# PRiME-project/PRiMEStereoMatch

Measured on AMD Instinct MI355X. Metric: cost-volume voxels/s (CVC+CVF+WTA), higher is better.
Workload: dtype f32; 1 GPU; synthetic 1920x1080 pair, D=256, float32 (BASELINE configs[3]); W=1920, H=1080, D=256, parallelism=1 GPU, kernel_variant=0, lr_check_on_gpu=False, batch=1, ranks=1, same_device=False, frames_in_flight=1

## Files before the change

### include/primesm_hip.h

```cpp
#ifndef PRIMESM_HIP_H
#define PRIMESM_HIP_H

#include <stddef.h>
#include <stdint.h>

#ifdef __cplusplus
extern "C" {
#endif

#define PSM_ABI_VERSION 1

typedef struct psm_ctx psm_ctx;

enum { PSM_F32 = 0, PSM_U8 = 1 };
enum { PSM_IMG_U8 = 0, PSM_IMG_F32 = 1 };
enum { PSM_LEFT = 0, PSM_RIGHT = 1 };
enum { PSM_STAGE_CVC = 0, PSM_STAGE_CVF = 1, PSM_STAGE_DISPSEL = 2, PSM_STAGE_PP = 3,
       PSM_STAGE_COUNT = 4 };
enum { PSM_K_PREP = 0, PSM_K_CVC = 1, PSM_K_GUIDE = 2, PSM_K_CVF_A = 3, PSM_K_CVF_B = 4,
       PSM_K_WTA = 5, PSM_K_MERGE = 6, PSM_K_BOX = 7, PSM_K_LRC = 8, PSM_K_CVF_F = 9, PSM_K_FGF = 10, PSM_K_WMF = 11,
       PSM_K_JWMF = 12, PSM_K_COUNT = 13 };
enum {
    PSM_OPT_ASYNC = 0,
    PSM_OPT_KERNEL_VARIANT = 1,
    PSM_OPT_PROFILE = 2,
    PSM_OPT_SEG_ROWS = 3,
    PSM_OPT_WAVES = 4,
    PSM_OPT_FLAGS = 5,
    PSM_OPT_GRAPH = 6,
    PSM_OPT_GATHER_STAGED = 7,
    PSM_OPT_FRAMES_IN_FLIGHT = 8
};

enum psm_flag {
    PSM_FLAG_MATERIALISE_COSTS = 128,
    PSM_FLAG_FGF_STORE = 4096,
    PSM_FLAG_STORE_FILTERED = 8192,
    PSM_FLAG_TWO_PHASE_ON = 1048576,
    PSM_FLAG_TWO_PHASE_OFF = 2097152,
    PSM_FLAG_WMF_DATAFLOW = 4194304,
    PSM_FLAG_WMF_TWO_SWEEPS = 8388608,
    PSM_FLAG_WMF_NO_CACHE = 16777216,
    PSM_FLAG_F32_TOL = 33554432,
    PSM_FLAG_FMA_SOLVE = 67108864,
    PSM_FLAGS_ALL = 128 | 4096 | 8192 | 1048576 | 2097152 | 4194304 | 8388608 | 16777216 | 33554432 | 67108864
};

int psm_device_count(void);

int psm_create(psm_ctx **out, int width, int height, int max_disp, int dtype, int device);

int psm_create_shard(psm_ctx **out, int width, int height, int max_disp, int d_begin, int d_end,
                     int dtype, int device);
int psm_create_shard_strided(psm_ctx **out, int width, int height, int max_disp, int d_first, int d_step,
// ... 189 lines not shown
```

### primestereomatch_amd/capi.py

```python
from __future__ import annotations

import ctypes as C
import os

_HERE = os.path.dirname(os.path.abspath(__file__))
LIB_PATH = os.path.join(_HERE, "lib", "libprimesm_hip.so")

PSM_F32, PSM_U8 = 0, 1
PSM_IMG_U8, PSM_IMG_F32 = 0, 1
PSM_LEFT, PSM_RIGHT = 0, 1
PSM_STAGE_CVC, PSM_STAGE_CVF, PSM_STAGE_DISPSEL, PSM_STAGE_PP = 0, 1, 2, 3
(PSM_K_PREP, PSM_K_CVC, PSM_K_GUIDE, PSM_K_CVF_A, PSM_K_CVF_B, PSM_K_WTA, PSM_K_MERGE, PSM_K_BOX,
 PSM_K_LRC, PSM_K_CVF_F, PSM_K_FGF, PSM_K_WMF, PSM_K_JWMF) = range(13)
(PSM_OPT_ASYNC, PSM_OPT_KERNEL_VARIANT, PSM_OPT_PROFILE, PSM_OPT_SEG_ROWS, PSM_OPT_WAVES, PSM_OPT_FLAGS, PSM_OPT_GRAPH,
 PSM_OPT_GATHER_STAGED, PSM_OPT_FRAMES_IN_FLIGHT) = range(9)
PSM_FLAG_MATERIALISE_COSTS, PSM_FLAG_FGF_STORE, PSM_FLAG_STORE_FILTERED = 128, 4096, 8192
PSM_FLAG_TWO_PHASE_ON, PSM_FLAG_TWO_PHASE_OFF = 1048576, 2097152
PSM_FLAG_WMF_DATAFLOW, PSM_FLAG_WMF_TWO_SWEEPS, PSM_FLAG_WMF_NO_CACHE = 4194304, 8388608, 16777216
PSM_FLAG_F32_TOL = 33554432
PSM_PP_LR_CHECK, PSM_PP_FILL, PSM_PP_WGT_MEDIAN = 1, 2, 4
PSM_FLAG_FMA_SOLVE = 67108864
PSM_SCORE_GIF, PSM_SCORE_SGM, PSM_SCORE_SGM_INT = 0, 1, 2
PSM_MASK_NONE, PSM_MASK_NONOCC, PSM_MASK_DISC = 0, 1, 2
PSM_SCORE_FLAT = 1
PSM_DEPTH_GIF, PSM_DEPTH_SGM = 0, 1
PSM_DEPTH_XYZ, PSM_DEPTH_Z, PSM_DEPTH_CLOUD = 1, 2, 4
PSM_DEPTH_USE_MASK = 1
PSM_DEPTH_VOID = 0x7FC00000
PSM_WLS_GIF, PSM_WLS_SGM = 0, 1
PSM_WLS_USE_MASK, PSM_WLS_CONFIDENCE = 1, 2
PSM_WLS_CONF_LR, PSM_WLS_CONF_VAR = 1, 2
PSM_WLS_VOID = 0x7FC00000


class Score(C.Structure):
    _fields_ = [("min_val", C.c_int32), ("max_val", C.c_int32), ("pixels", C.c_uint32), ("bad", C.c_uint32),
                ("err_sum", C.c_uint64), ("unit", C.c_int32), ("flags", C.c_uint32)]

# ... 179 lines not shown
```

### primestereomatch_amd/csrc/psm_api_core.cpp

```cpp
#include "psm_ctx.h"

#include <chrono>
#include <cstdarg>
#include <cstdio>
#include <cstring>

using namespace psm;

namespace {
std::string g_create_error;
}

namespace psm {

double now_us()
{
    using namespace std::chrono;
    return duration_cast<duration<double, std::micro>>(steady_clock::now().time_since_epoch()).count();
}

int fail(psm_ctx *c, const char *fmt, ...)
{
    char buf[512];
    va_list ap;
// ... 387 lines not shown
        if (value < 0) return fail(c, "psm_set_option: seg_rows %d < 0", value);
        c->march.seg_rows = value; return 0;
    case PSM_OPT_WAVES:
        if (value != 1 && value != 2 && value != 4 && value != 8) return fail(c, "psm_set_option: waves %d not in {1,2,4,8}", value);
        c->march.waves = value; return 0;
    case PSM_OPT_FLAGS:
        if (value & ~PSM_FLAGS_ALL) return fail(c, "psm_set_option: unknown flag bits 0x%x", value & ~PSM_FLAGS_ALL);
        if (c->dtype == PSM_U8) value &= ~(PSM_FLAG_FMA_SOLVE | PSM_FLAG_F32_TOL);
        if ((value & PSM_FLAG_F32_TOL) && (value & PSM_FLAG_FMA_SOLVE))
            return fail(c, "psm_set_option: PSM_FLAG_F32_TOL and PSM_FLAG_FMA_SOLVE exclude each other (one arithmetic variant at a time)");
        if ((value ^ c->march.flags) & PSM_FLAG_FMA_SOLVE) c->guid_rows = Rows{};
        c->march.flags = value; return 0;
    case PSM_OPT_GRAPH:
#ifdef PSM_EXPERIMENTS
        c->opt_graph = value != 0; return 0;
#else
        if (value != 0) return fail(c, "psm_set_option: PSM_OPT_GRAPH is not part of the product library (hipGraph replay of a batch measured slower than its plain launches)");
        return 0;
#endif
    case PSM_OPT_GATHER_STAGED: c->opt_gather_staged = value != 0; return 0;
    case PSM_OPT_FRAMES_IN_FLIGHT:
        if (value < 1 || value > 64) return fail(c, "psm_set_option: frames in flight %d not in [1, 64]", value);
        c->march.inflight = value; return 0;
    default: return fail(c, "psm_set_option: unknown option %d", option);
    }
}

int psm_set_stream(psm_ctx *c, void *hip_stream)
{
    if (!c) return 1;
    if (bind(c)) return 1;
    if (c->shared) return fail(c, "psm_set_stream: the context shares its streams with a batch (psm_share_streams)");
    PSM_HIP(c, hipStreamSynchronize(c->stream));
    c->stream = hip_stream ? (hipStream_t)hip_stream : c->own_stream;
    return 0;
}

int psm_synchronize(psm_ctx *c)
{
    if (!c) return 1;
    if (bind(c)) return 1;
    PSM_HIP(c, hipStreamSynchronize(c->stream));
    if (c->copy_stream) PSM_HIP(c, hipStreamSynchronize(c->copy_stream));
    if (c->down_stream && c->down_stream != c->copy_stream) PSM_HIP(c, hipStreamSynchronize(c->down_stream));
    return 0;
}
// ... 249 lines not shown
```

### primestereomatch_amd/csrc/psm_kernels.h

```cpp
#pragma once
#include <hip/hip_runtime.h>
#include <stdint.h>
#include "psm_live.h"
#include "psm_wm_sched.h"
#include "psm_wls_tab.h"

namespace psm {

struct Guidance {
    float4 *g1;
    float4 *g2;
    float4 *g3;
    float2 *g4;
};

struct March {
    int seg_rows;
    int waves;
    int flags;
    int dstep = 1;
    int inflight = 1;
    int ybeg = 0, yend = 0;
    int y0(int H) const { (void)H; return yend > ybeg ? ybeg : 0; }
    int y1(int H) const { return yend > ybeg ? yend : H; }
    int rows(int H) const { return y1(H) - y0(H); }
};

struct PcPair {
    const void *raw[2];
    Guidance g[2];
    uint8_t *p4[2];
    void *scratch;
    long long *keys;
    uint8_t *maps;
};
template <typename R> struct Recs { const R *host, *dev; int n; };
template <typename R, int N = 1> struct RecVal { R r[N]; };
template <typename R> using RecTab = const R *;
template <typename R> __device__ __forceinline__ const R &rec(const R *tab, unsigned i) { return tab[i]; }
template <typename R, int N> __device__ __forceinline__ const R &rec(const RecVal<R, N> &v, unsigned i) { return v.r[N == 1 ? 0 : i]; }
template <typename T>
__device__ __forceinline__ T *sgm_global(T *const &slot) { return (T *)*(__attribute__((address_space(1))) T *const *)(const void *)&slot; }
template <typename T> struct RecArg { using type = T; };
// ... 26 lines not shown
using PcTab = RecTab<PcPair>;
void launch_merge_batch(hipStream_t s, const Recs<PcPair> &q, int W, int H);

void launch_copy_bytes(hipStream_t s, void *dst, const void *src, size_t bytes);
void launch_range_f32(hipStream_t s, const float *p, size_t n, unsigned *out);
void launch_prep(hipStream_t s, const Recs<PcPair> &q, size_t pitch, int depth_f32, int W, int y0, int y1, bool u8_planes);
void launch_guidance(hipStream_t s, const Recs<PcPair> &q, int W, int H, int ybeg, int yend, bool fma, int src = 0, size_t pitch = 0);
void launch_cvc(hipStream_t s, const float4 *g1_base, const float4 *g1_other, float *vol, int W, int H,
                int d_begin, int Dloc, int right, int ybeg, int yend);
void launch_cvf_a(hipStream_t s, int variant, March m, const float *vol, float4 *ab, Guidance g, int W,
                  int H, int Dloc, int ybeg, int yend);
void launch_cvf_b_direct(hipStream_t s, const float4 *ab, float *vol, Guidance g, int W, int H, int Dloc);
void launch_cvf_fused(hipStream_t s, March m, const Recs<PcPair> &q, const float *vin, float *vout, int W, int H, int Dloc,
                      int ybeg, int yend, int d_begin, int cvc_mode, unsigned long long *ts = nullptr);
struct PcDev { int nxcd = 0, cus_per_xcd = 0; };
PcDev pc_dev();
enum { PC_STORE = 0, PC_PLANES = 1, PC_KEYS = 2, PC_BOTH = 4 };
struct PcPlan {
    int ngroups, nsegs, seg_rows, DC, nchunks, nbmax, nxcd;
    int cols;
    bool narrow;
    size_t rec_per_chunk;
    int rec_bytes;
    size_t scratch_bytes() const { return rec_per_chunk * (size_t)nchunks * rec_bytes; }
};
PcPlan pc_plan(int W, int rows, int Dloc, int seg_rows_opt, int form, int batch = 1, int inflight = 1);
PcPlan pc_plan_select(March m, int W, int H, int Dloc, int form, int npairs, bool batch);
int pc_seed_stride(int W, int rows, bool u8);
constexpr int PC_TS_SLOTS = 4096;
void launch_cvf_select(hipStream_t s, March m, const Recs<PcPair> &q, const float *vin, bool u8, int W, int H, int Dloc, int d_begin,
                       int cvc_mode, unsigned long long *ts = nullptr);
void launch_chunk_min(hipStream_t s, March m, const Recs<PcPair> &q, int W, int H, int Dloc);
void launch_cvf_select2(hipStream_t s, March m, const Recs<PcPair> &q, bool u8, int W, int H, int Dloc, int d_begin, unsigned long long *ts,
                        int sel, int step);
void launch_chunk_min2sides(hipStream_t s, March m, const Recs<PcPair> &q, int W, int H, int Dloc, bool to_maps, int d_begin, int sel, int step);
void launch_cvf_select_keys2(hipStream_t s, March m, const Recs<PcPair> &q, bool u8, int W, int H, int Dloc, int d_begin,
                             unsigned long long *ts, int sel, int step);
void launch_box8(hipStream_t s, int variant, March m, const float *vol, float *out, int W, int H, int Dloc);
void launch_wta(hipStream_t s, const float *vol, int W, int H, int d_begin, int Dloc, long long *keys,
                uint8_t *map);
void launch_merge(hipStream_t s, const long long *keys_all, size_t rank_stride, int nranks, int n,
                  uint8_t *map);

void launch_wgt_median(hipStream_t s, uint8_t *dis, const uint8_t *valid, const float4 *g1, int W, int H, int maxDis, int right,
                       int *nxt, int *prog, int *err);
struct WmSide {
// ... 261 lines not shown
```

### primestereomatch_amd/csrc/psm_pc.hip

```cpp
#include "psm_kernels.h"
#include "psm_cost.h"
#include "psm_dev.h"
#include "psm_live.h"
#include "../../include/primesm_hip.h"

#include <mutex>
#include <type_traits>

#include "psm_pc_debug.inc"

namespace psm {

typedef float f4v __attribute__((ext_vector_type(4)));

constexpr int PC_RING = 4;

template <int MODE, bool NARROW = false> struct PcLayout;
template <> struct PcLayout<0, false> { static constexpr int NA = 2, NB = 2, OUT_A = 52, OUT_B = 48, COLS = 96; };
template <> struct PcLayout<1, false> { static constexpr int NA = 2, NB = 2, OUT_A = 57, OUT_B = 54, COLS = 107; };
template <> struct PcLayout<2, false> : PcLayout<1, false> {};
template <> struct PcLayout<1, true> { static constexpr int NA = 1, NB = 1, OUT_A = 57, OUT_B = 50, COLS = 50; };
template <> struct PcLayout<2, true> : PcLayout<1, true> {};
constexpr int PC_K_LD_AUX = 0;
constexpr int PC_KEY_LD_AUX = 1;

typedef unsigned pc_u2 __attribute__((ext_vector_type(2)));
// ... 8 lines not shown
}
__device__ __forceinline__ float pc_load1_l2(__amdgpu_buffer_rsrc_t r, int voff, int soff)
{
    return __uint_as_float(__builtin_amdgcn_raw_buffer_load_b32(r, voff, soff, 16));
}
__device__ __forceinline__ float2 pc_load2(__amdgpu_buffer_rsrc_t r, int voff, int soff)
{
    const pc_u2 v = __builtin_amdgcn_raw_buffer_load_b64(r, voff, soff, 0);
    return make_float2(__uint_as_float(v.x), __uint_as_float(v.y));
}
__device__ __forceinline__ float4 pc_load4(__amdgpu_buffer_rsrc_t r, int voff, int soff)
{
    const pc_u4 v = __builtin_amdgcn_raw_buffer_load_b128(r, voff, soff, 0);
    return make_float4(__uint_as_float(v.x), __uint_as_float(v.y), __uint_as_float(v.z), __uint_as_float(v.w));
}

typedef unsigned pc_u3 __attribute__((ext_vector_type(3)));
__device__ __forceinline__ float3 pc_load3(__amdgpu_buffer_rsrc_t r, int voff, int soff)
{
    const pc_u3 v = __builtin_amdgcn_raw_buffer_load_b96(r, voff, soff, 0);
    return make_float3(__uint_as_float(v.x), __uint_as_float(v.y), __uint_as_float(v.z));
}

constexpr int PC_LIVE_MAX = 6;
struct PcLive {
    int on;
    int lo, full;
    int pre[2], nshort[2], tot[2];
    int cnt[2][PC_LIVE_MAX];
};
__host__ __device__ __forceinline__ int pc_live_count(const PcLive &lv, int side, int g)
{
    const int k = g - (side ? lv.pre[1] : lv.pre[0]), ns = side ? lv.nshort[1] : lv.nshort[0];
    int c = lv.full;
#pragma unroll
    for (int i = 0; i < PC_LIVE_MAX; ++i)
        if (i == k && i < ns) c = side ? lv.cnt[1][i] : lv.cnt[0][i];
    return c;
}
struct PcSel {
    int sel, step;
    int nxcd;
    int spread;
    unsigned long long rec_total;
    int dstep;
    PcLive live;
};
__device__ __forceinline__ int pc_spread(const PcSel &o, int n, int i)
{
    if (o.spread > 1) {
        int r = 0, base = 0;
        for (; r < o.spread; ++r) {
            const int cnt = (n - r + o.spread - 1) / o.spread;
            if (i < base + cnt) break;
            base += cnt;
        }
        i = (i - base) * o.spread + r;
    }
    return i;
}

template <bool VEC4, int CVC, int MODE, typename S, bool U8 = false, int VAR = 0, bool NARROW = false>
__global__ __launch_bounds__(64 * (PcLayout<MODE, NARROW>::NA + PcLayout<MODE, NARROW>::NB))
__attribute__((amdgpu_waves_per_eu(MODE == 2 ? 4 : 1, MODE == 2 ? 4 : 8)))
void k_cvf_pc(S src, const float *__restrict__ vin, float *__restrict__ vout, int W, int H, int Dloc, int ngroups, int nsegs, int seg_rows,
              int ybeg, int yend, int d_begin, int DC, int nbmax, PcSel dyn, unsigned long long *__restrict__ ts)
{
    constexpr bool TOL = VAR == 1, FMA = VAR == 2, TABLE = std::is_pointer<S>::value;
    static_assert(VAR >= 0 && VAR <= 2 && !(TOL && (U8 || MODE == 0)) && !(FMA && (U8 || TABLE)), "tolerance form: float select forms; FMA solve: float mode, single pair");
    static_assert(!TABLE || (CVC == 3 && MODE != 0), "batched launches: both volumes per launch, select forms");
    const bool right = CVC == 2 || (CVC == 3 && blockIdx.y == 1);
    const bool s1 = CVC == 3 && blockIdx.y == 1;
    const PcPair &pp = rec(src, blockIdx.z);
    const float4 *const G1 = s1 ? pp.g[1].g1 : pp.g[0].g1, *const G2 = s1 ? pp.g[1].g2 : pp.g[0].g2, *const G3 = s1 ? pp.g[1].g3 : pp.g[0].g3;
    const float2 *const G4 = s1 ? pp.g[1].g4 : pp.g[0].g4;
    const float4 *const Gother = s1 ? pp.g[0].g1 : pp.g[1].g1;
    if (U8) { vin = (const float *)pp.p4[0]; vout = (float *)pp.p4[1]; }
    float *const kcost = MODE == 1 ? (float *)((char *)pp.scratch + (s1 ? dyn.rec_total * 20 : 0))
                       : MODE == 2 ? (float *)(pp.keys + (s1 ? (size_t)W * H : 0)) : nullptr;
    unsigned *const kdisp = MODE == 1 ? (unsigned *)(kcost + 4 * dyn.rec_total) : nullptr;
    static_assert(!NARROW || (MODE != 0 && CVC == 3), "the narrow layout exists for the two-volume select forms");
    using L = PcLayout<MODE, NARROW>;
    constexpr int PC_NA = L::NA, PC_NB = L::NB, PC_OUT_A = L::OUT_A, PC_OUT_B = L::OUT_B, PC_COLS = L::COLS;
    constexpr int PC_MCOLS = PC_NA * PC_OUT_A;
    constexpr bool SCALED = MODE != 0;
    constexpr float QSCALE = SCALED ? 0x1p-12f : 1.0f;
#define PSM_BOX(N) (SCALED ? (float)(N) : box_out(N))
    static_assert(PC_MCOLS >= PC_COLS + 7 && PC_OUT_A <= 57 && PC_OUT_B <= 57 && (MODE != 0 || (PC_COLS % 4) == 0), "bad producer/consumer layout");
    __shared__ __attribute__((aligned(16))) float4 ring[PC_RING][4][PC_MCOLS];
    __shared__ __attribute__((aligned(16))) float qbuf[MODE == 0 ? 2 : 1][MODE == 0 ? 4 : 1][MODE == 0 ? PC_COLS : 4];
    int id = blockIdx.x;
    const int npairs = ngroups * nsegs;
    const PcLive &lv = dyn.live;
    const int ltot = s1 ? lv.tot[1] : lv.tot[0];
    const int nitems = nsegs * ltot;
    const int ipx = (nitems + dyn.nxcd - 1) / dyn.nxcd;
    const int xcd = id % dyn.nxcd, jj = id / dyn.nxcd;
    const int item = xcd * ipx + jj;
    if (jj >= ipx || item >= nitems) return;
    if (ts != nullptr && threadIdx.x == 0) {
        (void)__hip_atomic_fetch_min(ts, (unsigned long long)wall_clock64(), __ATOMIC_RELAXED, __HIP_MEMORY_SCOPE_AGENT);
        if (blockIdx.x == 0 && blockIdx.y == 0) ts[2 * PC_TS_SLOTS] = (unsigned long long)MODE;
    }
    const int seg = item / ltot;
    int g, gi = item - seg * ltot, gn = lv.full;
    {
        const int pre = s1 ? lv.pre[1] : lv.pre[0], ns = s1 ? lv.nshort[1] : lv.nshort[0];
        if (gi < pre * lv.full) { g = gi / lv.full; gi -= g * lv.full; }
        else {
            gi -= pre * lv.full;
            g = pre;
            bool found = false;
#pragma unroll
            for (int k = 0; k < PC_LIVE_MAX; ++k) {
                const int c = s1 ? lv.cnt[1][k] : lv.cnt[0][k];
                if (!found && k < ns) {
                    if (gi < c) { found = true; gn = c; }
                    else { gi -= c; ++g; }
                }
            }
            if (!found) { const int q = gi / lv.full; g += q; gi -= q * lv.full; }
        }
    }
    const int pair = seg * ngroups + g;
    const int ch = lv.lo + gi;
    const int sl0 = pc_sel_index(dyn.sel, dyn.step, MODE == 2 ? lv.lo + pc_spread(dyn, gn, gi) : ch);
    const int wave = __builtin_amdgcn_readfirstlane(threadIdx.x >> 6), lane = threadIdx.x & 63;
    const bool is_a = wave < PC_NA;
    const int xg = g * PC_COLS;
    const int xm0 = xg - 4;
    const int y0 = ybeg + seg * seg_rows, y1 = min(yend, y0 + seg_rows);
    const int mstart = max(0, y0 - 4);
    const int mend = min(H - 1, max(y1 + 2, 4 - y0));
    const int nbA = (mend - mstart + 1 + 3) >> 2;
    const int nf = (y1 - y0) + 7;
    const int nbB = (nf + 3) >> 2;
    const int iters = nbB + 3;
    const int i1 = ((lane + 1) & 63) << 2, i2 = ((lane + 2) & 63) << 2, i4 = ((lane + 4) & 63) << 2;
    (void)i1;
    const size_t HW = (size_t)H * W;

    PC_TRACE_BEGIN()
    int ds_lo = 0, ds_hi = MODE == 1 ? min(DC, Dloc - ch * DC) : 1;
    if (MODE == 1 && lv.on) {
        const PcOwn own = {1, d_begin, dyn.dstep, dyn.sel, dyn.step};
        while (ds_lo < ds_hi && pc_dead_at(own, right, xg, xg + PC_COLS - 1, W, ch * DC + ds_lo)) ++ds_lo;
        while (ds_hi > ds_lo && pc_dead_at(own, right, xg, xg + PC_COLS - 1, W, ch * DC + ds_hi - 1)) --ds_hi;
        if (ds_lo >= ds_hi) return;
    }
    bool first = true;
    int rb = 0;
    for (int ds = ds_lo; ds < ds_hi; ++ds) {
    const int sl = MODE == 1 ? pc_sel_index(dyn.sel, dyn.step, ch * DC + ds) : sl0;
    const bool last_slice = ds == ds_hi - 1;
// ... 376 lines not shown
        int gs = -1, ge = -1;
        for (int g = 0; g < ngroups; ++g) {
            const int xf = g * cols, xl = xf + cols - 1;
            const int L = pc_live_end(own, side, xf, xl, W, n);
            if ((L < n && !pc_dead_at(own, side, xf, xl, W, L)) || (L - 1 >= skip0 && pc_dead_at(own, side, xf, xl, W, L - 1))) return all;
            const int end = chunks ? (L + DC - 1) / DC : L, c = L > skip0 && end > lv.lo ? end - lv.lo : 0;
            lv.tot[side] += c;
            if (c == lv.full) continue;
            if (gs < 0) gs = g;
            ge = g;
        }
        if (gs < 0) continue;
        if (ge - gs + 1 > PC_LIVE_MAX) return all;
        lv.pre[side] = gs;
        lv.nshort[side] = ge - gs + 1;
        for (int g = gs; g <= ge; ++g) {
            const int L = pc_live_end(own, side, g * cols, g * cols + cols - 1, W, n), end = chunks ? (L + DC - 1) / DC : L;
            lv.cnt[side][g - gs] = L > skip0 && end > lv.lo ? end - lv.lo : 0;
        }
    }
    return lv;
}

PcPlan pc_plan(int W, int rows, int Dloc, int seg_rows_opt, int form, int batch, int inflight)
{
    const bool planes = (form & 3) == PC_PLANES, keys = (form & 3) == PC_KEYS;
    if (PSM_KNOB(planes ? "PSM_PC_SEGP" : "PSM_PC_SEGK", 0) > 0 && (planes || keys))
        seg_rows_opt = PSM_KNOB(planes ? "PSM_PC_SEGP" : "PSM_PC_SEGK", 0);
    const int sides = ((form & PC_BOTH) ? 2 : 1) * (batch > 1 ? batch : 1);
    const PcDev dev = pc_dev();
    PcPlan pl;
    pl.nxcd = dev.nxcd;
    constexpr int WIDE = PcLayout<1>::COLS, NARROW = PcLayout<1, true>::COLS;
    const bool select2 = (form & 3) != PC_STORE && (form & PC_BOTH);
    const int narrow_knob = PSM_KNOB("PSM_PC_NARROW", 0);
    pl.narrow = select2 && (narrow_knob ? narrow_knob == 1 : 2 * ((W + NARROW - 1) / NARROW) < 4 * ((W + WIDE - 1) / WIDE));
    const int cols = (form & 3) == PC_STORE ? PcLayout<0>::COLS : (pl.narrow ? NARROW : WIDE);
    pl.cols = cols;
    pl.ngroups = (W + cols - 1) / cols;
    const int kdiv = PSM_KNOB("PSM_PC_KDIV", rows < 128 ? 32 : 64);
    const int kmax = rows / kdiv > 1 ? rows / kdiv : 1;
    int dcs[5] = {1, 2, 4, 8, 16};
    int ndc = planes ? 5 : 1;
    if (planes && PSM_KNOB("PSM_PC_DC", 0) > 0) { dcs[0] = PSM_KNOB("PSM_PC_DC", 0); ndc = 1; }
    const long slots = PSM_KNOB("PSM_PC_SLOTS", (long)dev.cus_per_xcd * (keys ? 4 : 3) * (pl.narrow ? 2 : 1));
    const int conc = inflight > 1 ? inflight : 1;
    const int model_knob = PSM_KNOB("PSM_PC_MODEL", 0);
    const bool flow = model_knob ? model_knob == 1 : (sides * conc > 2 && (long)W * rows < 524288);
    auto cost_of = [&](int dc, int kk) -> long {
        const int nch = (Dloc + dc - 1) / dc;
        if (flow) {
            const double items = (double)sides * conc * pl.ngroups * kk * nch, len = dc * ((rows + kk - 1) / kk + 14) + 10.0;
            double c = items * len / ((double)slots * dev.nxcd) + 0.5 * len;
            if (planes && dc == 1) c *= 1.06;
            return (long)(c * 16.0);
        }
        const long per_xcd = ((long)sides * pl.ngroups * kk * nch + dev.nxcd - 1) / dev.nxcd;
        if (keys) {
            return (2 * ((per_xcd + slots - 1) / slots) + 3) * ((rows + kk - 1) / kk + 30) / 2;
        }
        const long rounds2 = 2 * ((per_xcd + slots - 1) / slots) + 1;
        long c = rounds2 * dc * ((rows + kk - 1) / kk + 14) / 2 + (planes ? 2L * sides * nch : 0);
        if (planes && dc == 1) c += (long)(0.06 * c * ((double)W * rows >= 2097152.0 ? 1.0 : (double)W * rows / 2097152.0));
        return c;
    };
    auto allowed = [&](int dc, int kk) { return (dc == dcs[0] || dc <= Dloc) && (seg_rows_opt <= 0 || kk == (rows + seg_rows_opt - 1) / seg_rows_opt); };
    long best = -1;
    for (int di = 0; di < ndc; ++di)
        for (int kk = 1; kk <= kmax && kk <= 32; ++kk)
            if (allowed(dcs[di], kk)) { const long c = cost_of(dcs[di], kk); if (best < 0 || c < best) best = c; }
    int bk = seg_rows_opt > 0 ? (rows + seg_rows_opt - 1) / seg_rows_opt : 1, bdc = dcs[0];
    for (int di = 0; di < ndc && best >= 0; ++di)
        for (int kk = 1; kk <= kmax && kk <= 32; ++kk)
            if (allowed(dcs[di], kk) && cost_of(dcs[di], kk) == best) { bk = kk; bdc = dcs[di]; di = ndc; break; }
    pl.seg_rows = seg_rows_opt > 0 ? seg_rows_opt : (rows + bk - 1) / bk;
    if (pl.seg_rows > rows) pl.seg_rows = rows;
    pl.nsegs = (rows + pl.seg_rows - 1) / pl.seg_rows;
    pl.DC = bdc;
    pl.nchunks = (Dloc + bdc - 1) / bdc;
    pl.nbmax = (pl.seg_rows + 7 + 3) / 4;
    pl.rec_per_chunk = (size_t)pl.ngroups * pl.nsegs * pl.nbmax * pl.cols;
    pl.rec_bytes = 20;
    return pl;
}

constexpr int PC_KEY_SPREAD = 4;

int pc_seed_stride(int W, int rows, bool u8)
{
    const int e = PSM_KNOB("PSM_PC_S", 0);
    if (e > 1) return e;
    if (rows < 200 || (u8 && (size_t)W * rows >= 1500000)) return 5;
    return 8;
}

static int pc_blocks(const PcPlan &pl, const PcLive &lv)
{
    const int items = pl.nsegs * (lv.tot[0] > lv.tot[1] ? lv.tot[0] : lv.tot[1]);
    return pl.nxcd * ((items + pl.nxcd - 1) / pl.nxcd);
}

struct PcArgs {
    Recs<PcPair> q;
    const float *vin;
    float *vout;
    int W, H, Dloc, ybeg, yend, d_begin;
    PcSel sel;
    unsigned long long *ts;
};

struct PcForm {
    int mode, cvc;
    bool u8;
    int var;
    bool narrow, vec4;
};

template <int V> using pc_int = std::integral_constant<int, V>;
template <int... Vs, class Fn> static void pc_pick(int v, Fn &&fn) { (void)((v == Vs && (fn(pc_int<Vs>{}), true)) || ...); }
template <class Fn> static void pc_pick_bool(bool b, Fn &&fn) { if (b) fn(std::true_type{}); else fn(std::false_type{}); }

static void pc_launch(hipStream_t s, const PcPlan &pl, dim3 grid, const PcArgs &a, const PcForm &f)
{
    using F = std::false_type;
    using T = std::true_type;
    const bool planes = f.mode == PC_PLANES;
    if (grid.x == 0) return;
    const PcVal val = {{a.q.host[0]}};
    const PcTab tab = a.q.dev;
    auto go = [&](auto V4, auto CV, auto MD, auto src, auto U, auto VR, auto NW) {
        using L = PcLayout<MD, NW>;
        hipLaunchKernelGGL(HIP_KERNEL_NAME(k_cvf_pc<V4, CV, MD, decltype(src), U, VR, NW>), grid, dim3(64 * (L::NA + L::NB)), 0, s, src, a.vin,
                           a.vout, a.W, a.H, a.Dloc, pl.ngroups, pl.nsegs, pl.seg_rows, a.ybeg, a.yend, a.d_begin, planes ? pl.DC : 1,
                           planes ? pl.nbmax : 0, a.sel, a.ts);
    };
    if (f.mode == PC_STORE)
        pc_pick_bool(f.vec4, [&](auto V4) { pc_pick<0, 1, 2>(f.cvc, [&](auto CV) {
            pc_pick<0, 2>(f.var, [&](auto VR) { go(V4, CV, pc_int<0>{}, val, F{}, VR, F{}); }); }); });
    else if (f.cvc != 3)
        pc_pick<0, 1, 2>(f.cvc, [&](auto CV) {
            if constexpr (CV != 0) if (f.u8) return go(F{}, CV, pc_int<1>{}, val, T{}, pc_int<0>{}, F{});
            pc_pick<0, 2>(f.var, [&](auto VR) { go(F{}, CV, pc_int<1>{}, val, F{}, VR, F{}); });
        });
    else
        pc_pick<1, 2>(f.mode, [&](auto MD) { pc_pick_bool(f.narrow, [&](auto NW) {
            if (tab) pc_pick_bool(f.u8, [&](auto U) { go(F{}, pc_int<3>{}, MD, tab, U, pc_int<0>{}, NW); });
            else if (f.u8) go(F{}, pc_int<3>{}, MD, val, T{}, pc_int<0>{}, NW);
            else pc_pick<0, 1, 2>(f.var, [&](auto VR) { go(F{}, pc_int<3>{}, MD, val, F{}, VR, NW); });
        }); });
}

static int pc_var(March m, bool u8)
{
    return u8 ? 0 : (m.flags & PSM_FLAG_FMA_SOLVE) ? 2 : (m.flags & PSM_FLAG_F32_TOL) ? 1 : 0;
}

static void pc_chunk_min(hipStream_t s, March m, const PcPlan &pl, int W, int H, int sides, const Recs<PcPair> &q, const PcLive &lv, bool to_maps)
{
    rec_launch(s, k_chunk_min<PcVal>, k_chunk_min<PcTab>, dim3((unsigned)((pl.rec_per_chunk + 255) / 256), sides, q.n),
               dim3(256), 0, q, pl.nchunks, pl.ngroups * pl.nsegs, pl.nbmax, pl.ngroups, pl.seg_rows, W, H, m.y0(H), m.y1(H), to_maps ? 1 : 0,
               pl.cols, lv);
}

void launch_cvf_fused(hipStream_t s, March m, const Recs<PcPair> &q, const float *vin, float *vout, int W, int H, int Dloc,
                      int ybeg, int yend, int d_begin, int cvc_mode, unsigned long long *ts)
{
    if (yend <= ybeg) return;
    const PcPlan pl = pc_plan(W, yend - ybeg, Dloc, m.seg_rows, PC_STORE);
    const PcLive lv = pc_live(W, pl.cols, pl.ngroups, Dloc, 1, false, PcOwn{});
    const PcArgs a = {q, vin, vout, W, H, Dloc, ybeg, yend, d_begin, PcSel{0, 1, pl.nxcd, 0, 0, 1, lv}, ts};
    const int cvc = cvc_mode == 1 || cvc_mode == 2 ? cvc_mode : 0;
    pc_launch(s, pl, dim3(pc_blocks(pl, lv)), a, {PC_STORE, cvc, false, (m.flags & PSM_FLAG_FMA_SOLVE) ? 2 : 0, false, (W & 3) == 0});
}

void launch_cvf_select(hipStream_t s, March m, const Recs<PcPair> &q, const float *vin, bool u8, int W, int H, int Dloc, int d_begin,
                       int cvc_mode, unsigned long long *ts)
{
    const PcPlan pl = pc_plan(W, m.rows(H), Dloc, m.seg_rows, PC_PLANES);
    const int cvc = cvc_mode == 1 || cvc_mode == 2 ? cvc_mode : 0;
    const PcLive lv = pc_live(W, pl.cols, pl.ngroups, Dloc, pl.DC, true, PcOwn{});
    const PcArgs a = {q, vin, nullptr, W, H, Dloc, m.y0(H), m.y1(H), d_begin, PcSel{0, 1, pl.nxcd, 0, pl.rec_per_chunk * pl.nchunks, 1, lv}, ts};
    pc_launch(s, pl, dim3(pc_blocks(pl, lv)), a, {PC_PLANES, cvc, u8 && cvc != 0, (m.flags & PSM_FLAG_FMA_SOLVE) ? 2 : 0, false, false});
}

void launch_chunk_min(hipStream_t s, March m, const Recs<PcPair> &q, int W, int H, int Dloc)
{
    const PcPlan pl = pc_plan(W, m.rows(H), Dloc, m.seg_rows, PC_PLANES);
    pc_chunk_min(s, m, pl, W, H, 1, q, pc_live(W, pl.cols, pl.ngroups, Dloc, pl.DC, true, PcOwn{}), false);
}

static PcOwn pc_own(March m, int d_begin, int sel, int step) { return PcOwn{1, d_begin, m.dstep, sel, step}; }
PcPlan pc_plan_select(March m, int W, int H, int Dloc, int form, int npairs, bool batch)
{
    return pc_plan(W, m.rows(H), Dloc, m.seg_rows, form | PC_BOTH, npairs, batch ? 1 : m.inflight);
}

void launch_cvf_select2(hipStream_t s, March m, const Recs<PcPair> &q, bool u8, int W, int H, int Dloc, int d_begin, unsigned long long *ts,
                        int sel, int step)
{
    const PcPlan pl = pc_plan_select(m, W, H, Dloc, PC_PLANES, q.n, q.dev != nullptr);
    const PcLive lv = pc_live(W, pl.cols, pl.ngroups, Dloc, pl.DC, true, pc_own(m, d_begin, sel, step));
    const PcArgs a = {q, nullptr, nullptr, W, H, Dloc, m.y0(H), m.y1(H), d_begin,
                      PcSel{sel, step, pl.nxcd, 0, pl.rec_per_chunk * pl.nchunks, m.dstep, lv}, ts};
    pc_launch(s, pl, dim3(pc_blocks(pl, lv), 2, q.n), a, {PC_PLANES, 3, u8, pc_var(m, u8), pl.narrow, false});
}

void launch_chunk_min2sides(hipStream_t s, March m, const Recs<PcPair> &q, int W, int H, int Dloc, bool to_maps, int d_begin, int sel, int step)
{
    const PcPlan pl = pc_plan_select(m, W, H, Dloc, PC_PLANES, q.n, q.dev != nullptr);
    const PcLive lv = pc_live(W, pl.cols, pl.ngroups, Dloc, pl.DC, true, pc_own(m, d_begin, sel, step));
    pc_chunk_min(s, m, pl, W, H, 2, q, lv, to_maps);
}

void launch_cvf_select_keys2(hipStream_t s, March m, const Recs<PcPair> &q, bool u8, int W, int H, int Dloc, int d_begin,
                             unsigned long long *ts, int sel, int step)
{
    const PcPlan pl = pc_plan_select(m, W, H, Dloc, PC_KEYS, q.n, q.dev != nullptr);
    const PcLive lv = pc_live(W, pl.cols, pl.ngroups, Dloc, 1, false, pc_own(m, d_begin, sel, step));
    const PcArgs a = {q, nullptr, nullptr, W, H, Dloc, m.y0(H), m.y1(H), d_begin,
                      PcSel{sel, step, pl.nxcd, PSM_KNOB("PSM_PC_SPREAD", PC_KEY_SPREAD), 0, m.dstep, lv}, ts};
    pc_launch(s, pl, dim3(pc_blocks(pl, lv), 2, q.n), a, {PC_KEYS, 3, u8, pc_var(m, u8), pl.narrow, false});
}

}

extern "C" int psm_debug_pc_dead(int right, int xfirst, int xlast, int W, int dg, int dprev)
{
    return psm::pc_dead(right, xfirst, xlast, W, dg, dprev) ? 1 : 0;
}

extern "C" int psm_debug_pc_items(int W, int rows, int nsl, int form, int d_begin, int dstep, int sel, int step, int *out)
{
    using namespace psm;
    if (!out || W < 1 || rows < 1 || nsl < 1 || dstep < 1 || form < PC_STORE || form > PC_KEYS) return 1;
    March m = {};
    m.dstep = dstep;
    m.yend = rows;
    PcOwn own = pc_own(m, d_begin, sel, step);
    if (form == PC_STORE) own.on = 0;
    const PcPlan pl = form == PC_STORE ? pc_plan(W, rows, nsl, 0, PC_STORE) : pc_plan_select(m, W, rows, nsl, form, 1, false);
    const bool chunks = form == PC_PLANES;
    const PcLive lv = pc_live(W, pl.cols, pl.ngroups, nsl, chunks ? pl.DC : 1, chunks, own);
    int slices[2] = {0, 0};
    for (int side = 0; side < 2; ++side)
        for (int g = 0; g < pl.ngroups; ++g)
            for (int j = 0; j < nsl; ++j)
                slices[side] += pc_dead_at(own, side, g * pl.cols, g * pl.cols + pl.cols - 1, W, j) ? 0 : 1;
    const int v[12] = {pl.ngroups, pl.nsegs, pl.DC, pl.cols, lv.tot[0], lv.tot[1], pl.ngroups * (chunks ? pl.nchunks : nsl),
                       slices[0], slices[1], pc_blocks(pl, lv), lv.lo, 0};
    for (int i = 0; i < 12; ++i) out[i] = v[i];
    return 0;
}

extern "C" int psm_debug_pc_group_items(int W, int rows, int nsl, int form, int d_begin, int dstep, int sel, int step, int side, int g,
                                        int *out)
{
    using namespace psm;
    if (!out || W < 1 || rows < 1 || nsl < 1 || dstep < 1 || form < PC_PLANES || form > PC_KEYS || side < 0 || side > 1 || g < 0) return 1;
    March m = {};
    m.dstep = dstep;
    m.yend = rows;
    const PcPlan pl = pc_plan_select(m, W, rows, nsl, form, 1, false);
    if (g >= pl.ngroups) return 1;
    const bool chunks = form == PC_PLANES;
    const PcLive lv = pc_live(W, pl.cols, pl.ngroups, nsl, chunks ? pl.DC : 1, chunks, pc_own(m, d_begin, sel, step));
    out[0] = lv.lo;
    out[1] = pc_live_count(lv, side, g);
    return 0;
}
```

Measured before the change: 167.9 billion voxels/s.

## Schedule key-select blocks with a two-tier segment split to balance the tail round

Adds a host-computed schedule for the single-pair key-select CVF launch. Both sides are merged into one flattened item list, spread across XCDs, and a tail set of items is split into finer row segments so the last wave of blocks fills the slots. A cost model picks between the plain split and the two-tier split, and a new option or env knob can force a cut. The kernel decodes its item from the schedule, which adds per-block index math and shorter segments with extra halo rows in the tail.

```diff
diff --git a/include/primesm_hip.h b/include/primesm_hip.h
--- a/include/primesm_hip.h
+++ b/include/primesm_hip.h
@@ -29,7 +29,8 @@
     PSM_OPT_FLAGS = 5,
     PSM_OPT_GRAPH = 6,
     PSM_OPT_GATHER_STAGED = 7,
-    PSM_OPT_FRAMES_IN_FLIGHT = 8
+    PSM_OPT_FRAMES_IN_FLIGHT = 8,
+    PSM_OPT_KEY_CUT = 9
 };
 
 enum psm_flag {
diff --git a/primestereomatch_amd/capi.py b/primestereomatch_amd/capi.py
--- a/primestereomatch_amd/capi.py
+++ b/primestereomatch_amd/capi.py
@@ -13,7 +13,15 @@
 (PSM_K_PREP, PSM_K_CVC, PSM_K_GUIDE, PSM_K_CVF_A, PSM_K_CVF_B, PSM_K_WTA, PSM_K_MERGE, PSM_K_BOX,
  PSM_K_LRC, PSM_K_CVF_F, PSM_K_FGF, PSM_K_WMF, PSM_K_JWMF) = range(13)
 (PSM_OPT_ASYNC, PSM_OPT_KERNEL_VARIANT, PSM_OPT_PROFILE, PSM_OPT_SEG_ROWS, PSM_OPT_WAVES, PSM_OPT_FLAGS, PSM_OPT_GRAPH,
- PSM_OPT_GATHER_STAGED, PSM_OPT_FRAMES_IN_FLIGHT) = range(9)
+ PSM_OPT_GATHER_STAGED, PSM_OPT_FRAMES_IN_FLIGHT, PSM_OPT_KEY_CUT) = range(10)
+
+
+def key_cut(kb, kt, T):
+    assert 1 <= kb <= 255 and 1 <= kt <= 4095 and 0 <= T <= 2047
+    return kb | kt << 8 | T << 20
+
+
+
 PSM_FLAG_MATERIALISE_COSTS, PSM_FLAG_FGF_STORE, PSM_FLAG_STORE_FILTERED = 128, 4096, 8192
 PSM_FLAG_TWO_PHASE_ON, PSM_FLAG_TWO_PHASE_OFF = 1048576, 2097152
 PSM_FLAG_WMF_DATAFLOW, PSM_FLAG_WMF_TWO_SWEEPS, PSM_FLAG_WMF_NO_CACHE = 4194304, 8388608, 16777216
diff --git a/primestereomatch_amd/csrc/psm_api_core.cpp b/primestereomatch_amd/csrc/psm_api_core.cpp
--- a/primestereomatch_amd/csrc/psm_api_core.cpp
+++ b/primestereomatch_amd/csrc/psm_api_core.cpp
@@ -433,6 +433,10 @@
     case PSM_OPT_FRAMES_IN_FLIGHT:
         if (value < 1 || value > 64) return fail(c, "psm_set_option: frames in flight %d not in [1, 64]", value);
         c->march.inflight = value; return 0;
+    case PSM_OPT_KEY_CUT:
+        if (value < 0 || (value != 0 && ((value & 255) == 0 || ((value >> 8) & 4095) == 0)))
+            return fail(c, "psm_set_option: key cut 0x%x is not 0 or k_b | k_t << 8 | T << 20 with k_b, k_t >= 1", value);
+        c->march.key_cut = value; return 0;
     default: return fail(c, "psm_set_option: unknown option %d", option);
     }
 }
diff --git a/primestereomatch_amd/csrc/psm_kernels.h b/primestereomatch_amd/csrc/psm_kernels.h
--- a/primestereomatch_amd/csrc/psm_kernels.h
+++ b/primestereomatch_amd/csrc/psm_kernels.h
@@ -19,6 +19,7 @@
     int waves;
     int flags;
     int dstep = 1;
+    int key_cut = 0;
     int inflight = 1;
     int ybeg = 0, yend = 0;
     int y0(int H) const { (void)H; return yend > ybeg ? ybeg : 0; }
@@ -91,6 +92,8 @@
     bool narrow;
     size_t rec_per_chunk;
     int rec_bytes;
+    int slots, kdiv;
+    bool rounds;
     size_t scratch_bytes() const { return rec_per_chunk * (size_t)nchunks * rec_bytes; }
 };
 PcPlan pc_plan(int W, int rows, int Dloc, int seg_rows_opt, int form, int batch = 1, int inflight = 1);
diff --git a/primestereomatch_amd/csrc/psm_pc.hip b/primestereomatch_amd/csrc/psm_pc.hip
--- a/primestereomatch_amd/csrc/psm_pc.hip
+++ b/primestereomatch_amd/csrc/psm_pc.hip
@@ -2,6 +2,7 @@
 #include "psm_cost.h"
 #include "psm_dev.h"
 #include "psm_live.h"
+#include "psm_sched.h"
 #include "../../include/primesm_hip.h"
 
 #include <mutex>
@@ -56,13 +57,6 @@
     return make_float3(__uint_as_float(v.x), __uint_as_float(v.y), __uint_as_float(v.z));
 }
 
-constexpr int PC_LIVE_MAX = 6;
-struct PcLive {
-    int on;
-    int lo, full;
-    int pre[2], nshort[2], tot[2];
-    int cnt[2][PC_LIVE_MAX];
-};
 __host__ __device__ __forceinline__ int pc_live_count(const PcLive &lv, int side, int g)
 {
     const int k = g - (side ? lv.pre[1] : lv.pre[0]), ns = side ? lv.nshort[1] : lv.nshort[0];
@@ -80,7 +74,7 @@
     int dstep;
     PcLive live;
 };
-__device__ __forceinline__ int pc_spread(const PcSel &o, int n, int i)
+__host__ __device__ __forceinline__ int pc_spread(const PcSel &o, int n, int i)
 {
     if (o.spread > 1) {
         int r = 0, base = 0;
@@ -98,13 +92,16 @@
 __global__ __launch_bounds__(64 * (PcLayout<MODE, NARROW>::NA + PcLayout<MODE, NARROW>::NB))
 __attribute__((amdgpu_waves_per_eu(MODE == 2 ? 4 : 1, MODE == 2 ? 4 : 8)))
 void k_cvf_pc(S src, const float *__restrict__ vin, float *__restrict__ vout, int W, int H, int Dloc, int ngroups, int nsegs, int seg_rows,
-              int ybeg, int yend, int d_begin, int DC, int nbmax, PcSel dyn, unsigned long long *__restrict__ ts)
+              int ybeg, int yend, int d_begin, int DC, int nbmax, PcSel dyn, unsigned long long *__restrict__ ts, PcSched sch)
 {
     constexpr bool TOL = VAR == 1, FMA = VAR == 2, TABLE = std::is_pointer<S>::value;
+    constexpr bool SCHED = MODE == 2 && !TABLE;
+    PcItem it = {};
+    if (SCHED && !pc_sched_item(sch, dyn.live, blockIdx.x, it)) return;
     static_assert(VAR >= 0 && VAR <= 2 && !(TOL && (U8 || MODE == 0)) && !(FMA && (U8 || TABLE)), "tolerance form: float select forms; FMA solve: float mode, single pair");
     static_assert(!TABLE || (CVC == 3 && MODE != 0), "batched launches: both volumes per launch, select forms");
-    const bool right = CVC == 2 || (CVC == 3 && blockIdx.y == 1);
-    const bool s1 = CVC == 3 && blockIdx.y == 1;
+    const bool right = CVC == 2 || (CVC == 3 && (SCHED ? it.side == 1 : blockIdx.y == 1));
+    const bool s1 = CVC == 3 && (SCHED ? it.side == 1 : blockIdx.y == 1);
     const PcPair &pp = rec(src, blockIdx.z);
     const float4 *const G1 = s1 ? pp.g[1].g1 : pp.g[0].g1, *const G2 = s1 ? pp.g[1].g2 : pp.g[0].g2, *const G3 = s1 ? pp.g[1].g3 : pp.g[0].g3;
     const float2 *const G4 = s1 ? pp.g[1].g4 : pp.g[0].g4;
@@ -131,14 +128,15 @@
     const int ipx = (nitems + dyn.nxcd - 1) / dyn.nxcd;
     const int xcd = id % dyn.nxcd, jj = id / dyn.nxcd;
     const int item = xcd * ipx + jj;
-    if (jj >= ipx || item >= nitems) return;
+    if (!SCHED && (jj >= ipx || item >= nitems)) return;
     if (ts != nullptr && threadIdx.x == 0) {
         (void)__hip_atomic_fetch_min(ts, (unsigned long long)wall_clock64(), __ATOMIC_RELAXED, __HIP_MEMORY_SCOPE_AGENT);
         if (blockIdx.x == 0 && blockIdx.y == 0) ts[2 * PC_TS_SLOTS] = (unsigned long long)MODE;
     }
     const int seg = item / ltot;
     int g, gi = item - seg * ltot, gn = lv.full;
-    {
+    if (SCHED) { g = it.g; gi = it.gi; gn = it.gn; }
+    else {
         const int pre = s1 ? lv.pre[1] : lv.pre[0], ns = s1 ? lv.nshort[1] : lv.nshort[0];
         if (gi < pre * lv.full) { g = gi / lv.full; gi -= g * lv.full; }
         else {
@@ -163,7 +161,7 @@
     const bool is_a = wave < PC_NA;
     const int xg = g * PC_COLS;
     const int xm0 = xg - 4;
-    const int y0 = ybeg + seg * seg_rows, y1 = min(yend, y0 + seg_rows);
+    const int y0 = ybeg + (SCHED ? it.y0 : seg * seg_rows), y1 = SCHED ? ybeg + it.y1 : min(yend, y0 + seg_rows);
     const int mstart = max(0, y0 - 4);
     const int mend = min(H - 1, max(y1 + 2, 4 - y0));
     const int nbA = (mend - mstart + 1 + 3) >> 2;
@@ -586,13 +584,12 @@
     return lv;
 }
 
-PcPlan pc_plan(int W, int rows, int Dloc, int seg_rows_opt, int form, int batch, int inflight)
+static PcPlan pc_plan_on(PcDev dev, long slots_opt, int W, int rows, int Dloc, int seg_rows_opt, int form, int batch, int inflight)
 {
     const bool planes = (form & 3) == PC_PLANES, keys = (form & 3) == PC_KEYS;
     if (PSM_KNOB(planes ? "PSM_PC_SEGP" : "PSM_PC_SEGK", 0) > 0 && (planes || keys))
         seg_rows_opt = PSM_KNOB(planes ? "PSM_PC_SEGP" : "PSM_PC_SEGK", 0);
     const int sides = ((form & PC_BOTH) ? 2 : 1) * (batch > 1 ? batch : 1);
-    const PcDev dev = pc_dev();
     PcPlan pl;
     pl.nxcd = dev.nxcd;
     constexpr int WIDE = PcLayout<1>::COLS, NARROW = PcLayout<1, true>::COLS;
@@ -607,7 +604,7 @@
     int dcs[5] = {1, 2, 4, 8, 16};
     int ndc = planes ? 5 : 1;
     if (planes && PSM_KNOB("PSM_PC_DC", 0) > 0) { dcs[0] = PSM_KNOB("PSM_PC_DC", 0); ndc = 1; }
-    const long slots = PSM_KNOB("PSM_PC_SLOTS", (long)dev.cus_per_xcd * (keys ? 4 : 3) * (pl.narrow ? 2 : 1));
+    const long slots = slots_opt > 0 ? slots_opt : PSM_KNOB("PSM_PC_SLOTS", (long)dev.cus_per_xcd * (keys ? 4 : 3) * (pl.narrow ? 2 : 1));
     const int conc = inflight > 1 ? inflight : 1;
     const int model_knob = PSM_KNOB("PSM_PC_MODEL", 0);
     const bool flow = model_knob ? model_knob == 1 : (sides * conc > 2 && (long)W * rows < 524288);
@@ -645,7 +642,63 @@
     pl.nbmax = (pl.seg_rows + 7 + 3) / 4;
     pl.rec_per_chunk = (size_t)pl.ngroups * pl.nsegs * pl.nbmax * pl.cols;
     pl.rec_bytes = 20;
+    pl.slots = (int)slots;
+    pl.kdiv = kdiv;
+    pl.rounds = !flow && seg_rows_opt <= 0;
     return pl;
+}
+
+PcPlan pc_plan(int W, int rows, int Dloc, int seg_rows_opt, int form, int batch, int inflight)
+{
+    return pc_plan_on(pc_dev(), 0, W, rows, Dloc, seg_rows_opt, form, batch, inflight);
+}
+
+static int pc_seg_rows(int rows, int k) { return (rows + k - 1) / k; }
+static int pc_seg_count(int rows, int k) { const int r = pc_seg_rows(rows, k); return (rows + r - 1) / r; }
+static long pc_key_cost2(const PcSched &s, long slots)
+{
+    const long n = (s.ncomb + s.nxcd - 1) / s.nxcd, nt = n < s.T ? n : s.T, nb = n - nt;
+    const long rb = (nb * s.kb + slots - 1) / slots, rt = (nt * s.kt + slots - 1) / slots;
+    return nt == 0 ? (2 * rb + 3) * (s.rows_b + 30) : 2 * rb * (s.rows_b + 30) + (2 * rt + 3) * (s.rows_t + 30);
+}
+PcSched pc_key_sched(const PcPlan &pl, const PcLive &lv, int rows, int cut)
+{
+    PcSched s = {};
+    s.nxcd = pl.nxcd;
+    s.ncomb = lv.tot[0] + lv.tot[1];
+    s.tot0 = lv.tot[0];
+    s.rows = rows;
+    auto with = [&](int kb, int kt, long T) {
+        PcSched c = s;
+        c.T = (int)T;
+        c.kb = pc_seg_count(rows, kb);
+        c.rows_b = pc_seg_rows(rows, kb);
+        c.kt = T > 0 ? pc_seg_count(rows, kt) : c.kb;
+        c.rows_t = T > 0 ? pc_seg_rows(rows, kt) : c.rows_b;
+        return c;
+    };
+    const long n = (s.ncomb + s.nxcd - 1) / s.nxcd, slots = pl.slots > 0 ? pl.slots : 1;
+    cut = PSM_KNOB("PSM_PC_KEYCUT", cut);
+    if (cut > 0) {
+        const int kb = cut & 255, kt = (cut >> 8) & 4095, T = (cut >> 20) & 2047;
+        auto clamp = [&](int k) { return k < 1 ? 1 : (k > rows ? rows : k); };
+        return with(clamp(kb), clamp(kt), T == 2047 || T > n ? n : T);
+    }
+    PcSched best = with(pl.nsegs, pl.nsegs, 0);
+    if (!pl.rounds || PSM_KNOB("PSM_PC_TAIL", 1) == 2) return best;
+    const int kb = best.kb, kmax = rows / pl.kdiv > 1 ? rows / pl.kdiv : 1;
+    const long rb = n * kb / slots, over = n * kb - rb * slots;
+    int kt = 3 * kb < kmax ? 3 * kb : kmax;
+    while (kt > kb && pc_seg_count(rows, kt) != kt) --kt;
+    if (rb < 1 || 3 * over < 2 * slots || kt <= kb) return best;
+    const PcSched c = with(kb, kt, n - rb * slots / kb);
+    return pc_key_cost2(c, slots) < pc_key_cost2(best, slots) ? c : best;
+}
+static int pc_sched_blocks(const PcSched &s)
+{
+    int m = 0;
+    for (int x = 0; x < s.nxcd; ++x) m = pc_sched_items(s, x) > m ? pc_sched_items(s, x) : m;
+    return s.nxcd * m;
 }
 
 constexpr int PC_KEY_SPREAD = 4;
@@ -671,6 +724,7 @@
     int W, H, Dloc, ybeg, yend, d_begin;
     PcSel sel;
     unsigned long long *ts;
+    PcSched sch;
 };
 
 struct PcForm {
@@ -696,7 +750,7 @@
         using L = PcLayout<MD, NW>;
         hipLaunchKernelGGL(HIP_KERNEL_NAME(k_cvf_pc<V4, CV, MD, decltype(src), U, VR, NW>), grid, dim3(64 * (L::NA + L::NB)), 0, s, src, a.vin,
                            a.vout, a.W, a.H, a.Dloc, pl.ngroups, pl.nsegs, pl.seg_rows, a.ybeg, a.yend, a.d_begin, planes ? pl.DC : 1,
-                           planes ? pl.nbmax : 0, a.sel, a.ts);
+                           planes ? pl.nbmax : 0, a.sel, a.ts, a.sch);
     };
     if (f.mode == PC_STORE)
         pc_pick_bool(f.vec4, [&](auto V4) { pc_pick<0, 1, 2>(f.cvc, [&](auto CV) {
@@ -732,7 +786,7 @@
     if (yend <= ybeg) return;
     const PcPlan pl = pc_plan(W, yend - ybeg, Dloc, m.seg_rows, PC_STORE);
     const PcLive lv = pc_live(W, pl.cols, pl.ngroups, Dloc, 1, false, PcOwn{});
-    const PcArgs a = {q, vin, vout, W, H, Dloc, ybeg, yend, d_begin, PcSel{0, 1, pl.nxcd, 0, 0, 1, lv}, ts};
+    const PcArgs a = {q, vin, vout, W, H, Dloc, ybeg, yend, d_begin, PcSel{0, 1, pl.nxcd, 0, 0, 1, lv}, ts, PcSched{}};
     const int cvc = cvc_mode == 1 || cvc_mode == 2 ? cvc_mode : 0;
     pc_launch(s, pl, dim3(pc_blocks(pl, lv)), a, {PC_STORE, cvc, false, (m.flags & PSM_FLAG_FMA_SOLVE) ? 2 : 0, false, (W & 3) == 0});
 }
@@ -743,7 +797,7 @@
     const PcPlan pl = pc_plan(W, m.rows(H), Dloc, m.seg_rows, PC_PLANES);
     const int cvc = cvc_mode == 1 || cvc_mode == 2 ? cvc_mode : 0;
     const PcLive lv = pc_live(W, pl.cols, pl.ngroups, Dloc, pl.DC, true, PcOwn{});
-    const PcArgs a = {q, vin, nullptr, W, H, Dloc, m.y0(H), m.y1(H), d_begin, PcSel{0, 1, pl.nxcd, 0, pl.rec_per_chunk * pl.nchunks, 1, lv}, ts};
+    const PcArgs a = {q, vin, nullptr, W, H, Dloc, m.y0(H), m.y1(H), d_begin, PcSel{0, 1, pl.nxcd, 0, pl.rec_per_chunk * pl.nchunks, 1, lv}, ts, PcSched{}};
     pc_launch(s, pl, dim3(pc_blocks(pl, lv)), a, {PC_PLANES, cvc, u8 && cvc != 0, (m.flags & PSM_FLAG_FMA_SOLVE) ? 2 : 0, false, false});
 }
 
@@ -765,7 +819,7 @@
     const PcPlan pl = pc_plan_select(m, W, H, Dloc, PC_PLANES, q.n, q.dev != nullptr);
     const PcLive lv = pc_live(W, pl.cols, pl.ngroups, Dloc, pl.DC, true, pc_own(m, d_begin, sel, step));
     const PcArgs a = {q, nullptr, nullptr, W, H, Dloc, m.y0(H), m.y1(H), d_begin,
-                      PcSel{sel, step, pl.nxcd, 0, pl.rec_per_chunk * pl.nchunks, m.dstep, lv}, ts};
+                      PcSel{sel, step, pl.nxcd, 0, pl.rec_per_chunk * pl.nchunks, m.dstep, lv}, ts, PcSched{}};
     pc_launch(s, pl, dim3(pc_blocks(pl, lv), 2, q.n), a, {PC_PLANES, 3, u8, pc_var(m, u8), pl.narrow, false});
 }
 
@@ -781,9 +835,12 @@
 {
     const PcPlan pl = pc_plan_select(m, W, H, Dloc, PC_KEYS, q.n, q.dev != nullptr);
     const PcLive lv = pc_live(W, pl.cols, pl.ngroups, Dloc, 1, false, pc_own(m, d_begin, sel, step));
+    const bool single = q.dev == nullptr;
+    const PcSched sch = single ? pc_key_sched(pl, lv, m.rows(H), m.key_cut) : PcSched{};
     const PcArgs a = {q, nullptr, nullptr, W, H, Dloc, m.y0(H), m.y1(H), d_begin,
-                      PcSel{sel, step, pl.nxcd, PSM_KNOB("PSM_PC_SPREAD", PC_KEY_SPREAD), 0, m.dstep, lv}, ts};
-    pc_launch(s, pl, dim3(pc_blocks(pl, lv), 2, q.n), a, {PC_KEYS, 3, u8, pc_var(m, u8), pl.narrow, false});
+                      PcSel{sel, step, pl.nxcd, PSM_KNOB("PSM_PC_SPREAD", PC_KEY_SPREAD), 0, m.dstep, lv}, ts, sch};
+    pc_launch(s, pl, single ? dim3(pc_sched_blocks(sch), 1, q.n) : dim3(pc_blocks(pl, lv), 2, q.n), a,
+              {PC_KEYS, 3, u8, pc_var(m, u8), pl.narrow, false});
 }
 
 }
@@ -810,8 +867,9 @@
         for (int g = 0; g < pl.ngroups; ++g)
             for (int j = 0; j < nsl; ++j)
                 slices[side] += pc_dead_at(own, side, g * pl.cols, g * pl.cols + pl.cols - 1, W, j) ? 0 : 1;
-    const int v[12] = {pl.ngroups, pl.nsegs, pl.DC, pl.cols, lv.tot[0], lv.tot[1], pl.ngroups * (chunks ? pl.nchunks : nsl),
-                       slices[0], slices[1], pc_blocks(pl, lv), lv.lo, 0};
+    const PcSched sch = form == PC_KEYS ? pc_key_sched(pl, lv, rows, 0) : PcSched{};
+    const int v[12] = {pl.ngroups, form == PC_KEYS ? sch.kb : pl.nsegs, pl.DC, pl.cols, lv.tot[0], lv.tot[1], pl.ngroups * (chunks ? pl.nchunks : nsl),
+                       slices[0], slices[1], form == PC_KEYS ? pc_sched_blocks(sch) : pc_blocks(pl, lv), lv.lo, 0};
     for (int i = 0; i < 12; ++i) out[i] = v[i];
     return 0;
 }
@@ -832,3 +890,33 @@
     out[1] = pc_live_count(lv, side, g);
     return 0;
 }
+
+extern "C" int psm_debug_pc_key_schedule(int W, int rows, int nsl, int d_begin, int dstep, int sel, int step, int nxcd, int slots, int cut,
+                                         int *out, int cap)
+{
+    using namespace psm;
+    if (W < 1 || rows < 1 || nsl < 1 || dstep < 1 || nxcd < 1 || slots < 1 || cut < 0 || sel < 0 || sel > 2 || (sel && step < 2) || (!out && cap > 0)) return -1;
+    March m = {};
+    m.dstep = dstep;
+    m.yend = rows;
+    const PcPlan pl = pc_plan_on(PcDev{nxcd, 1}, slots, W, rows, nsl, 0, PC_KEYS | PC_BOTH, 1, 1);
+    const PcLive lv = pc_live(W, pl.cols, pl.ngroups, nsl, 1, false, pc_own(m, d_begin, sel, step));
+    const PcSched s = pc_key_sched(pl, lv, rows, cut);
+    const PcSel dyn = {sel, step, nxcd, PC_KEY_SPREAD, 0, dstep, lv};
+    const int blocks = pc_sched_blocks(s), need = 8 + 5 * blocks;
+    if (cap < 8) return need;
+    const int head[8] = {blocks, s.kb, s.rows_b, s.kt, s.rows_t, s.T, s.ncomb, (int)pc_key_cost2(s, slots)};
+    for (int i = 0; i < 8; ++i) out[i] = head[i];
+    if (cap < need) return need;
+    for (int b = 0; b < blocks; ++b) {
+        PcItem it = {};
+        int *o = out + 8 + 5 * b;
+        if (!pc_sched_item(s, lv, b, it)) { o[0] = -1; o[1] = o[2] = o[3] = o[4] = 0; continue; }
+        o[0] = it.side;
+        o[1] = it.g;
+        o[2] = lv.lo + pc_spread(dyn, it.gn, it.gi);
+        o[3] = it.y0;
+        o[4] = it.y1;
+    }
+    return need;
+}
diff --git a/primestereomatch_amd/csrc/psm_sched.h b/primestereomatch_amd/csrc/psm_sched.h
--- /dev/null
+++ b/primestereomatch_amd/csrc/psm_sched.h
@@ -0,0 +1,82 @@
+#pragma once
+
+#include "psm_live.h"
+
+namespace psm {
+
+constexpr int PC_LIVE_MAX = 6;
+struct PcLive {
+    int on;
+    int lo, full;
+    int pre[2], nshort[2], tot[2];
+    int cnt[2][PC_LIVE_MAX];
+};
+
+struct PcSched {
+    int nxcd;
+    int ncomb, tot0;
+    int T;
+    int kb, rows_b;
+    int kt, rows_t;
+    int rows;
+};
+struct PcItem {
+    int side, g;
+    int gi, gn;
+    int y0, y1;
+};
+
+PSM_LIVE_FN int pc_sched_share(const PcSched &s, int x) { return (x + 1) * s.ncomb / s.nxcd - x * s.ncomb / s.nxcd; }
+PSM_LIVE_FN int pc_sched_items(const PcSched &s, int x)
+{
+    const int n = pc_sched_share(s, x), nt = n < s.T ? n : s.T;
+    return (n - nt) * s.kb + nt * s.kt;
+}
+
+PSM_LIVE_FN void pc_live_locate(const PcLive &lv, int side, int i, int &g, int &gi, int &gn)
+{
+    const int pre = side ? lv.pre[1] : lv.pre[0], ns = side ? lv.nshort[1] : lv.nshort[0];
+    gi = i;
+    gn = lv.full;
+    if (gi < pre * lv.full) { g = gi / lv.full; gi -= g * lv.full; }
+    else {
+        gi -= pre * lv.full;
+        g = pre;
+        bool found = false;
+#if defined(__HIPCC__)
+#pragma unroll
+#endif
+        for (int k = 0; k < PC_LIVE_MAX; ++k) {
+            const int c = side ? lv.cnt[1][k] : lv.cnt[0][k];
+            if (!found && k < ns) {
+                if (gi < c) { found = true; gn = c; }
+                else { gi -= c; ++g; }
+            }
+        }
+        if (!found) { const int q = gi / lv.full; g += q; gi -= q * lv.full; }
+    }
+}
+
+PSM_LIVE_FN bool pc_sched_item(const PcSched &s, const PcLive &lv, int block, PcItem &it)
+{
+    const int x = block % s.nxcd, j = block / s.nxcd;
+    const int c0 = x * s.ncomb / s.nxcd, n = (x + 1) * s.ncomb / s.nxcd - c0;
+    const int nt = n < s.T ? n : s.T, nb = n - nt;
+    int c, seg, sr;
+    if (j < nb * s.kb) { seg = j / nb; c = j - seg * nb; sr = s.rows_b; }
+    else {
+        const int t = j - nb * s.kb;
+        if (t >= nt * s.kt) return false;
+        seg = t / nt;
+        c = nb + t - seg * nt;
+        sr = s.rows_t;
+    }
+    c += c0;
+    it.side = c >= s.tot0 ? 1 : 0;
+    pc_live_locate(lv, it.side, it.side ? c - s.tot0 : c, it.g, it.gi, it.gn);
+    it.y0 = seg * sr;
+    it.y1 = it.y0 + sr < s.rows ? it.y0 + sr : s.rows;
+    return true;
+}
+
+}
```

Result: no change. 169.1 billion voxels/s, median of 6 (+0.7%).
